# esw0116/DynaVSR

Measured on AMD Instinct MI355X. Metric: inner-loop frames/sec/GPU (EDVR-M x4, 5x3x180x320): forward leg = BASELINE.json configs[1]; the inner MAML step and the per-frame pipeline are `inner_step` / `per_frame_pipeline`, higher is better.
Workload: dtype f32; 1 GPU; EDVR-M x4 forward (PCD deformable alignment + TSA fusion + reconstruction), clips of 1x5x3x180x320 -> 3x720x1280 (BASELINE.json configs[1]); one step = 2 clip(s) per GPU, one per HIP stream (adapt.super_resolve_video); clips_in_flight_per_gpu=2

## Files before the change

dynavsr_amd/csrc/conv2d_wino5.hip:

```cpp
#include <type_traits>

#include "common.h"
#include "kernels.h"
#include "small_grid.h"

namespace dvsr {

#ifdef DVSR_CONV_TRACE
#define W5_STAMP(i)                                                                                       \
  do {                                                                                                    \
    if (a.trace && threadIdx.x == 0) a.trace[(size_t)blockIdx.x * 64 + (i)] = __builtin_readcyclecounter(); \
  } while (0)
#else
#define W5_STAMP(i) \
  do {              \
  } while (0)
#endif

typedef float w5f2 __attribute__((ext_vector_type(2)));
typedef __bf16 w5bf8 __attribute__((ext_vector_type(8)));
typedef __bf16 w5bf2 __attribute__((ext_vector_type(2)));
typedef unsigned w5u4 __attribute__((ext_vector_type(4)));

constexpr int W5_PCH = 18 * 2 * 3 * 256;

template <int TC>
struct Wino5Shape {
  static constexpr int CC = 8, NTILE = 32, TRW = NTILE / TC, NT = 768;
  static constexpr int OH = 4 * TRW, OW = 4 * TC;
  static constexpr int IH = OH + 2, RP = OW + 8, GR = RP / 4;
  static constexpr int NG = CC * IH * GR;
  static constexpr int NI = (NG + NT - 1) / NT;
  static constexpr int RAWPAD = NI * NT * 4;
  static constexpr int VIMG = 36 * 3 * 32 * 4;
  static constexpr int XCH = 6 * 16 * 64 * 4;
  static constexpr int LOOP = 2 * RAWPAD + 2 * VIMG;
  static constexpr size_t LDS_BYTES = (size_t)(LOOP > XCH ? LOOP : XCH) * sizeof(float);
};

constexpr int w5_waitcnt(int vm, int lgkm) { return (vm & 15) | (7 << 4) | ((lgkm & 15) << 8) | ((vm >> 4) << 14); }

__device__ __forceinline__ unsigned w5_cvt_pk(float a, float b) {
  return __builtin_bit_cast(unsigned, __builtin_convertvector(w5f2{a, b}, w5bf2));
}
__device__ __forceinline__ void w5_dma16(__amdgpu_buffer_rsrc_t rs, float* lds, unsigned voff, unsigned soff) {
  __builtin_amdgcn_raw_ptr_buffer_load_lds(rs, (__attribute__((address_space(3))) void*)lds, 16, voff, soff, 0, 0);
}
__device__ __forceinline__ __amdgpu_buffer_rsrc_t w5_rsrc(const float* base, int num_records) {
  return __builtin_amdgcn_make_buffer_rsrc(const_cast<float*>(base), 0, num_records, 0x00020000);
}

__global__ void pack_weights_wino5_kernel(PackTable t) {
  const PackEntry& e = t.e[blockIdx.y];
  if (e.layout != PackLayout::WINO_F4) return;
  __bf16* const P16 = reinterpret_cast<__bf16*>(e.P);
  const size_t total = (size_t)e.ncb * e.nchunks * 512;
  constexpr double G[6][3] = {{1.0 / 4, 0, 0},          {-1.0 / 6, -1.0 / 6, -1.0 / 6}, {-1.0 / 6, 1.0 / 6, -1.0 / 6},
                              {1.0 / 24, 1.0 / 12, 1.0 / 6}, {1.0 / 24, -1.0 / 12, 1.0 / 6}, {0, 0, 1}};
  for (size_t i = blockIdx.x * (size_t)blockDim.x + threadIdx.x; i < total; i += (size_t)gridDim.x * blockDim.x) {
    const int c8 = (int)(i & 7), col = (int)((i >> 3) & 63);
    const size_t ck = i >> 9;
    const int k = (int)(ck % e.nchunks), cb = (int)(ck / e.nchunks);
    const int co = cb * 64 + col, ci = k * 8 + c8;
    double g[3][3];
    const bool ok = co < e.Cout && ci < e.Ctot;
    const float* src = !e.wt ? e.w + ((size_t)co * (e.w_ctot ? e.w_ctot : e.Ctot) + (e.w_ctot ? e.w_coff : 0) + ci) * 9
                             : e.w + ((size_t)ci * e.w_ctot + e.w_coff + co) * 9;
#pragma unroll
    for (int tap = 0; tap < 9; ++tap) g[tap / 3][tap % 3] = ok ? (double)src[e.wt ? 8 - tap : tap] : 0.0;
    double c[6][3];
#pragma unroll
    for (int xi = 0; xi < 6; ++xi)
#pragma unroll
      for (int b = 0; b < 3; ++b) c[xi][b] = G[xi][0] * g[0][b] + G[xi][1] * g[1][b] + G[xi][2] * g[2][b];
    const int mh = col >> 5, c32 = col & 31;
    __bf16* dst = P16 + ck * (size_t)(2 * W5_PCH) + (size_t)mh * 1536 + (size_t)c32 * 8 + c8;
#pragma unroll
    for (int xi = 0; xi < 6; ++xi)
#pragma unroll
      for (int nu = 0; nu < 6; ++nu) {
        const float u = (float)(c[xi][0] * G[nu][0] + c[xi][1] * G[nu][1] + c[xi][2] * G[nu][2]);
        const __bf16 h = (__bf16)u;
        const float r1 = u - (float)h;
        const __bf16 m = (__bf16)r1;
        const __bf16 l = (__bf16)(r1 - (float)m);
        __bf16* d = dst + (size_t)(xi * 3 + (nu >> 1)) * 3072;
        if (nu & 1) { d[512] = m; d[768] = h; d[1024] = l; }
        else { d[0] = h; d[256] = m; d[1280] = l; }
      }
  }
}

int pack_weights_wino5_run(const PackTable& t, hipStream_t st) {
  hipLaunchKernelGGL(pack_weights_wino5_kernel, dim3(64, t.n), dim3(256), 0, st, t);
  return check_launch("pack_weights_wino5_kernel");
}

template <int TC, bool RES, bool R16, bool PRE>
__global__ __launch_bounds__(1024) void conv2d_wino5_kernel(ConvK2 a) {
  static_assert(!PRE || (R16 && !RES), "the addend is read by the sixteen-reader epilogue, never beside a residual");
  using Sh = Wino5Shape<TC>;
  constexpr int IH = Sh::IH, RP = Sh::RP, GR = Sh::GR;
  constexpr int CHF = IH * RP;
  constexpr int QF = 768 * 4;
  extern __shared__ __attribute__((aligned(16))) float smem[];
  float* const raw0 = smem;
  unsigned* const vimg0 = reinterpret_cast<unsigned*>(smem + 2 * Sh::RAWPAD);

  const int id = blockIdx.x;
  const int q_ = id >> 3;
  const int cbi = q_ % a.ncb;
  const int j_ = q_ / a.ncb;
  const int tile = (id & 7) * a.tiles_per_xcd + j_;
  if (j_ >= a.tiles_per_xcd || tile >= a.ntiles) return;
  const int tx_ = tile % a.tiles_x;
  const int t2 = tile / a.tiles_x;
  const int ty_ = t2 % a.tiles_y;
  const int n = t2 / a.tiles_y;
  const int oy0 = ty_ * Sh::OH, ox0 = tx_ * Sh::OW;

  const int tid = threadIdx.x, lane = tid & 63;
  const int wave = __builtin_amdgcn_readfirstlane(tid >> 6);
  const int lo = lane & 31, hi = lane >> 5;
  const size_t HW = (size_t)a.H * a.W;
  auto fence = [&]() __attribute__((always_inline)) { __builtin_amdgcn_sched_barrier(0); };
  auto lds_barrier = [&]() __attribute__((always_inline)) {
    asm volatile("s_waitcnt lgkmcnt(0)" ::: "memory");
    __builtin_amdgcn_s_barrier();
    asm volatile("" ::: "memory");
  };
  W5_STAMP(0);
#ifdef DVSR_CONV_TRACE
  if (a.trace && threadIdx.x == 0) a.trace[(size_t)blockIdx.x * 64 + 60] = __builtin_amdgcn_s_memrealtime();
#endif

  auto read16 = [&](int m) __attribute__((always_inline)) {
    int le = lane;
    asm volatile("" : "+v"(le));
    const int rq_r = wave & 3, cp_r = wave >> 2;
    const float* const xr = smem + (rq_r * 64 + le) * 4 + cp_r;
    const int lo_e = le & 31, hi_e = le >> 5;
    const int trow_e = lo_e / TC, tcol_e = lo_e - trow_e * TC;
    const int oy = oy0 + 4 * trow_e, ox = ox0 + 4 * tcol_e;
    const size_t HWo = (size_t)a.Ho * a.Wo;
    const float slope = a.act == ACT_LRELU ? 0.1f : (a.act == ACT_RELU ? 0.f : 1.f);
    const float* bias = wset_ptr(a.bias, a.b_gs, n, a.wdiv);
    const int co0 = cbi * 64 + m * 32 + 8 * rq_r + 4 * hi_e + cp_r;
    f32x4 pr[4];
    if constexpr (PRE) {
      const bool live = oy < a.Ho && ox < a.Wo && co0 < a.Cout;
      const float* pre = a.pre + (size_t)(n / a.pre_bdiv) * a.pre_bs + (size_t)co0 * HWo + (size_t)oy * a.Wo + ox;
#pragma unroll
      for (int i = 0; i < 4; ++i)
        pr[i] = (live && oy + i < a.Ho) ? *reinterpret_cast<const f32x4*>(pre + (size_t)i * a.Wo) : f32x4{0.f, 0.f, 0.f, 0.f};
    }
    float y[4][4];
#pragma unroll
    for (int j = 0; j < 4; ++j) {
      float z[6];
#pragma unroll
      for (int x = 0; x < 6; ++x) z[x] = xr[(x * 16 + j * 4) * 256];
      const float sa = z[1] + z[2], da = z[1] - z[2];
      const float sb = z[3] + z[4], db = z[3] - z[4];
      y[0][j] = z[0] + sa + sb;
      y[1][j] = __builtin_fmaf(2.f, db, da);
      y[2][j] = __builtin_fmaf(4.f, sb, sa);
      y[3][j] = __builtin_fmaf(8.f, db, da) + z[5];
    }
    const bool px_ok = oy < a.Ho && ox < a.Wo;
    const int nrow = a.Ho - oy < 4 ? a.Ho - oy : 4;
    if (px_ok && co0 < a.Cout) {
      const float b0 = bias ? bias[co0] : 0.f;
      const size_t base = ((size_t)n * a.Cout + co0) * HWo + (size_t)oy * a.Wo + ox;
      f32x4 rr[4];
      if constexpr (RES) {
#pragma unroll
        for (int i = 0; i < 4; ++i)
          rr[i] = i < nrow ? *reinterpret_cast<const f32x4*>(a.res + base + (size_t)i * a.Wo) : f32x4{0.f, 0.f, 0.f, 0.f};
      }
#pragma unroll
      for (int i = 0; i < 4; ++i) {
        if (i >= nrow) break;
        f32x4 v;
#pragma unroll
        for (int j = 0; j < 4; ++j) {
          float v0 = y[i][j] + b0;
          if constexpr (PRE) v0 += pr[i][j];
          v[j] = fmaxf(v0, v0 * slope);
        }
        if constexpr (RES) v += rr[i];
        *reinterpret_cast<f32x4*>(a.y + base + (size_t)i * a.Wo) = v;
      }
    }
  };

  if (wave >= 12) {
    const int pw = wave - 12, ptid = tid - 768;
    const float* x0n = a.x0 + (size_t)n * a.x0_bs;
    const float* x1n = a.c1 ? a.x1 + (size_t)(n / a.x1_bdiv) * a.x1_bs : x0n;
    static_assert(IH * GR * 4 == 720, "a channel quad is 720 groups");
    unsigned hoff[3];
#pragma unroll
    for (int jj = 0; jj < 3; ++jj) {
      const int L = jj * 256 + ptid;
      const int cq = L / (IH * GR), rr = L - cq * (IH * GR);
      const int iy = rr / GR, g = rr - iy * GR;
      const int gy = oy0 - 1 + iy, gx = ox0 - 4 + 4 * g;
      const bool live = L < 4 * IH * GR;
      const bool ok = live && (unsigned)gy < (unsigned)a.H && (unsigned)gx < (unsigned)a.W;
      hoff[jj] = ok ? (unsigned)(((size_t)cq * HW + (size_t)gy * a.W + gx) * 4) : 0x80000000u;
      if (live && !ok) {
#pragma unroll
        for (int bb = 0; bb < 4; ++bb) *reinterpret_cast<f32x4*>(raw0 + (bb >> 1) * Sh::RAWPAD + (bb & 1) * QF + L * 4) = f32x4{0.f, 0.f, 0.f, 0.f};
      }
    }
    const unsigned chunk_bytes = (unsigned)(Sh::CC * HW * 4), quad_bytes = (unsigned)(4 * HW * 4);
    auto issue_raw = [&](int k) __attribute__((always_inline)) {
      const bool live = k < a.nchunks;
      const bool second = k * Sh::CC >= a.c0;
      const unsigned soff = live ? (unsigned)(second ? k - a.c0 / Sh::CC : k) * chunk_bytes : 0u;
      const __amdgpu_buffer_rsrc_t rs = w5_rsrc(second ? x1n : x0n, live ? 0x7fffffff : 0);
      float* dst = raw0 + (k & 1) * Sh::RAWPAD + 256 * pw;
#pragma unroll
      for (int jj = 0; jj < 3; ++jj) {
        w5_dma16(rs, dst + jj * 1024, hoff[jj], soff);
        w5_dma16(rs, dst + QF + jj * 1024, hoff[jj], soff + quad_bytes);
      }
    };
    const int ptile = 8 * pw + (lane & 7), ppair = (lane >> 3) & 3;
    const int trow_t = ptile / TC, tcol_t = ptile - trow_t * TC;
    const int pch = 2 * ppair + hi;
    const float* prd = raw0 + (pch >> 2) * QF + (pch & 3) * CHF + 4 * trow_t * RP + 4 * tcol_t;
    unsigned* vw12 = vimg0 + (hi ? 2 : 1) * 6 * 384 + ptile * 4 + ppair;
    unsigned* vw34 = vimg0 + (hi ? 4 : 3) * 6 * 384 + ptile * 4 + ppair;
    unsigned* vw05 = vimg0 + (hi ? 5 : 0) * 6 * 384 + ptile * 4 + ppair;
    auto ld_row = [&](float (&d)[6], int row) __attribute__((always_inline)) {
      const float* p = prd + row * RP;
      const w5f2 l2 = *reinterpret_cast<const w5f2*>(p + 2);
      const f32x4 m4 = *reinterpret_cast<const f32x4*>(p + 4);
      const w5f2 h2 = *reinterpret_cast<const w5f2*>(p + 8);
      d[0] = l2[1]; d[1] = m4[0]; d[2] = m4[1]; d[3] = m4[2]; d[4] = m4[3]; d[5] = h2[0];
    };
    auto colpass = [&](const float (&r)[6], float (&v)[6]) __attribute__((always_inline)) {
      v[0] = __builtin_fmaf(4.f, r[0], __builtin_fmaf(-5.f, r[2], r[4]));
      v[5] = __builtin_fmaf(4.f, r[1], __builtin_fmaf(-5.f, r[3], r[5]));
      const float e1 = __builtin_fmaf(-4.f, r[2], r[4]), o1 = __builtin_fmaf(-4.f, r[1], r[3]);
      v[1] = e1 + o1; v[2] = e1 - o1;
      const float e2 = r[4] - r[2], o2 = r[3] - r[1];
      v[3] = __builtin_fmaf(2.f, o2, e2); v[4] = __builtin_fmaf(-2.f, o2, e2);
    };
    auto finish_pair = [&](const float (&ra)[6], const float (&rb)[6], unsigned* vw) __attribute__((always_inline)) {
      float va[6], vb[6];
      colpass(ra, va);
      colpass(rb, vb);
#pragma unroll
      for (int v = 0; v < 6; ++v) {
        const auto s0 = __builtin_amdgcn_permlane32_swap(__builtin_bit_cast(unsigned, va[v]), __builtin_bit_cast(unsigned, vb[v]), false, false);
        const unsigned u0 = s0[0], u1 = s0[1];
        const float v0 = __builtin_bit_cast(float, u0), v1 = __builtin_bit_cast(float, u1);
        const unsigned h = w5_cvt_pk(v0, v1);
        const float r0 = v0 - __builtin_bit_cast(float, h << 16), r1 = v1 - __builtin_bit_cast(float, h & 0xffff0000u);
        const unsigned m = w5_cvt_pk(r0, r1);
        const float q0 = r0 - __builtin_bit_cast(float, m << 16), q1 = r1 - __builtin_bit_cast(float, m & 0xffff0000u);
        unsigned* d = vw + v * 384;
#ifdef W5_NOVW
        d[0] = h ^ m ^ w5_cvt_pk(q0, q1);
#else
        d[0] = h; d[128] = m; d[256] = w5_cvt_pk(q0, q1);
#endif
      }
    };
    auto produce = [&]() __attribute__((always_inline)) {
      float d0[6], d1[6], d2[6], d3[6], d4[6], d5[6];
      ld_row(d1, 1); ld_row(d2, 2); ld_row(d3, 3); ld_row(d4, 4);
      ld_row(d0, 0); ld_row(d5, 5);
      float ra[6], rb[6];
#pragma unroll
      for (int j = 0; j < 6; ++j) {
        const float e = __builtin_fmaf(-4.f, d2[j], d4[j]), o = __builtin_fmaf(-4.f, d1[j], d3[j]);
        ra[j] = e + o; rb[j] = e - o;
      }
      finish_pair(ra, rb, vw12);
      fence();
#pragma unroll
      for (int j = 0; j < 6; ++j) {
        const float e = d4[j] - d2[j], o = d3[j] - d1[j];
        ra[j] = __builtin_fmaf(2.f, o, e); rb[j] = __builtin_fmaf(-2.f, o, e);
      }
      finish_pair(ra, rb, vw34);
      fence();
#pragma unroll
      for (int j = 0; j < 6; ++j) {
        ra[j] = __builtin_fmaf(4.f, d0[j], __builtin_fmaf(-5.f, d2[j], d4[j]));
        rb[j] = __builtin_fmaf(4.f, d1[j], __builtin_fmaf(-5.f, d3[j], d5[j]));
      }
      finish_pair(ra, rb, vw05);
    };
    issue_raw(0);
    issue_raw(1);
    __builtin_amdgcn_s_waitcnt(w5_waitcnt(6, 0));
    __builtin_amdgcn_s_barrier();
    asm volatile("" ::: "memory");
    produce();
    __builtin_amdgcn_s_waitcnt(w5_waitcnt(0, 0));
    __builtin_amdgcn_s_barrier();
    asm volatile("" ::: "memory");
    int vstep = Sh::VIMG, rstep = Sh::RAWPAD;
    vw12 += vstep; vw34 += vstep; vw05 += vstep; prd += rstep;
    __builtin_amdgcn_s_setprio(3);
    for (int k = 0; k < a.nchunks; ++k) {

#ifndef W5_NODMA
      issue_raw(k + 2);
#endif
#ifndef W5_NOPROD
      if (k + 1 < a.nchunks) produce();
#endif
      __builtin_amdgcn_s_waitcnt(w5_waitcnt(0, 0));
      __builtin_amdgcn_s_barrier();
      asm volatile("" ::: "memory");
      vw12 -= vstep; vw34 -= vstep; vw05 -= vstep; prd -= rstep;
      vstep = -vstep; rstep = -rstep;
    }
    if constexpr (R16) {
      __builtin_amdgcn_s_setprio(0);
      lds_barrier();
      lds_barrier(); read16(0);
      lds_barrier();
      lds_barrier(); read16(1);
    } else {
      lds_barrier(); lds_barrier(); lds_barrier(); lds_barrier();
    }
    return;
  }
  {
    const int cxi = wave % 6, cmh = wave / 6;
    f32x16 acc[6];
#pragma unroll
    for (int v = 0; v < 6; ++v)
#pragma unroll
      for (int r = 0; r < 16; ++r) acc[v][r] = 0.f;
    const float* wp_cb = wset_ptr(a.wp, a.w_gs, n, a.wdiv) + (size_t)cbi * a.nchunks * W5_PCH;
    const __amdgpu_buffer_rsrc_t wrsrc = w5_rsrc(wp_cb, -1);
    const unsigned avoff = (unsigned)(lane * 16);
    const int asb = (cxi * 3 * 2 + cmh) * 3072;
    f32x4 AF[3];
    auto gldA = [&](auto g_, int k) __attribute__((always_inline)) {
      constexpr int G = decltype(g_)::value;
#ifdef W5_NOA
      if (k > 0 || G > 2) return;
#endif
      const int soff = k * (W5_PCH * 4) + asb + (G / 3) * 6144 + (G % 3) * 1024;
      AF[G % 3] = __builtin_bit_cast(f32x4, __builtin_amdgcn_raw_buffer_load_b128(wrsrc, (int)avoff, soff, 0));
    };
    auto blend = [&](f32x4& x, const f32x4& l, bool keep) __attribute__((always_inline)) {
#pragma unroll
      for (int r = 0; r < 4; ++r) x[r] = keep ? x[r] : l[r];
    };
    const unsigned* vrd = vimg0 + cxi * 6 * 384 + lo * 4;
    const unsigned* vrd_lh = vrd + (hi ? 0 : 256);
    const unsigned* vrd_hl = vrd + (hi ? 256 : 0);
    w5u4 BF[2];
    auto ldB = [&](auto f_) __attribute__((always_inline)) {
      constexpr int F = decltype(f_)::value, NU = F / 3, W = F % 3;
      if constexpr (W == 0) BF[F & 1] = *reinterpret_cast<const w5u4*>(vrd + NU * 384);
      else if constexpr (W == 1) BF[F & 1] = *reinterpret_cast<const w5u4*>(vrd + NU * 384 + 128);
      else if constexpr (NU & 1) BF[F & 1] = *reinterpret_cast<const w5u4*>(vrd_hl + NU * 384);
      else BF[F & 1] = *reinterpret_cast<const w5u4*>(vrd_lh + NU * 384);
    };
    auto mma = [&](f32x16& c, const f32x4& av, const w5u4& bv) __attribute__((always_inline)) {
#ifdef W5_NOMMA
      c[0] += av[0] * __builtin_bit_cast(float, bv[0]);
      return;
#endif
      c = __builtin_amdgcn_mfma_f32_32x32x16_bf16(__builtin_bit_cast(w5bf8, av), __builtin_bit_cast(w5bf8, bv), c, 0, 0, 0);
    };
    static_for<0, 3>([&](auto g_) __attribute__((always_inline)) { gldA(g_, 0); });
    __builtin_amdgcn_s_barrier();
    asm volatile("" ::: "memory");
    __builtin_amdgcn_s_barrier();
    asm volatile("" ::: "memory");
    int vstep = Sh::VIMG;
    for (int k = 0; k < a.nchunks; ++k) {
      ldB(std::integral_constant<int, 0>{}); ldB(std::integral_constant<int, 1>{});
      const int knext = k + 1 < a.nchunks ? k + 1 : k;
      static_for<0, 18>([&](auto f_) __attribute__((always_inline)) {
        constexpr int F = decltype(f_)::value, NU = F / 3, I = F % 3;
        constexpr int XS = NU & 1;
        mma(acc[NU], AF[XS], BF[F & 1]);
#ifdef W5_NOBR
        if constexpr (false)
#else
        if constexpr (F + 2 < 18)
#endif
          ldB(std::integral_constant<int, (F + 2 < 18 ? F + 2 : 0)>{});
        if constexpr (I == 1) {
          blend(AF[XS], AF[2], (NU & 1) ? hi != 0 : hi == 0);
          if constexpr ((NU & 1) && NU < 5) gldA(std::integral_constant<int, 3 * ((NU < 5 ? NU : 1) / 2) + 5>{}, k);
          if constexpr (NU == 5) gldA(std::integral_constant<int, 2>{}, knext);
        }
        if constexpr (I == 2) {
          if constexpr (NU < 4) gldA(std::integral_constant<int, 3 * ((NU < 4 ? NU : 0) / 2) + 3 + (NU & 1)>{}, k);
          else gldA(std::integral_constant<int, (NU & 1)>{}, knext);
        }
        fence();
      });
      lds_barrier();
      if (k < 16) W5_STAMP(3 + k);
      vrd += vstep; vrd_lh += vstep; vrd_hl += vstep;
      vstep = -vstep;
    }
  W5_STAMP(40);

  int lane_e = lane;
  asm volatile("" : "+v"(lane_e));
  f32x16 Z[4];
#pragma unroll
  for (int r = 0; r < 16; ++r) {
    const float sa = acc[1][r] + acc[2][r], da = acc[1][r] - acc[2][r];
    const float sb = acc[3][r] + acc[4][r], db = acc[3][r] - acc[4][r];
    Z[0][r] = acc[0][r] + sa + sb;
    Z[1][r] = __builtin_fmaf(2.f, db, da);
    Z[2][r] = __builtin_fmaf(4.f, sb, sa);
    Z[3][r] = __builtin_fmaf(8.f, db, da) + acc[5][r];
  }
  float* const xw = smem + (cxi * 16 * 64 + lane_e) * 4;
  const int rq_r = wave & 3, cp_r = wave >> 2;
  const float* const xr = smem + (rq_r * 64 + lane_e) * 4 + cp_r * 2;
  const int lo_e = lane_e & 31, hi_e = lane_e >> 5;
  const int trow_e = lo_e / TC, tcol_e = lo_e - trow_e * TC;
  const int oy = oy0 + 4 * trow_e, ox = ox0 + 4 * tcol_e;
  const size_t HWo = (size_t)a.Ho * a.Wo;
  const float slope = a.act == ACT_LRELU ? 0.1f : (a.act == ACT_RELU ? 0.f : 1.f);
  const float* bias = wset_ptr(a.bias, a.b_gs, n, a.wdiv);
  W5_STAMP(50);
  lds_barrier();
  W5_STAMP(51);
#pragma unroll 1
  for (int m = 0; m < 2; ++m) {
    if (cmh == m) {
#pragma unroll
      for (int j = 0; j < 4; ++j)
#pragma unroll
        for (int rq = 0; rq < 4; ++rq)
          *reinterpret_cast<f32x4*>(xw + (j * 4 + rq) * 256) = f32x4{Z[j][4 * rq], Z[j][4 * rq + 1], Z[j][4 * rq + 2], Z[j][4 * rq + 3]};
    }
    W5_STAMP(52 + 4 * m);
    lds_barrier();
    W5_STAMP(53 + 4 * m);
    if constexpr (R16) read16(m);
    else if (wave < 8) {
      const int co0 = cbi * 64 + m * 32 + 8 * rq_r + 4 * hi_e + 2 * cp_r;
      float y[2][4][4];
#pragma unroll
      for (int j = 0; j < 4; ++j) {
        w5f2 z[6];
#pragma unroll
        for (int x = 0; x < 6; ++x) z[x] = *reinterpret_cast<const w5f2*>(xr + (x * 16 + j * 4) * 256);
#pragma unroll
        for (int c = 0; c < 2; ++c) {
          const float sa = z[1][c] + z[2][c], da = z[1][c] - z[2][c];
          const float sb = z[3][c] + z[4][c], db = z[3][c] - z[4][c];
          y[c][0][j] = z[0][c] + sa + sb;
          y[c][1][j] = __builtin_fmaf(2.f, db, da);
          y[c][2][j] = __builtin_fmaf(4.f, sb, sa);
          y[c][3][j] = __builtin_fmaf(8.f, db, da) + z[5][c];
        }
      }
      const bool px_ok = oy < a.Ho && ox < a.Wo;
      const int nrow = a.Ho - oy < 4 ? a.Ho - oy : 4;
      if (px_ok && co0 < a.Cout) {
        const bool two = co0 + 1 < a.Cout;
        const float b0 = bias ? bias[co0] : 0.f, b1 = (bias && two) ? bias[co0 + 1] : 0.f;
#pragma unroll
        for (int i = 0; i < 4; ++i)
#pragma unroll
          for (int j = 0; j < 4; ++j) {
            const float v0 = y[0][i][j] + b0, v1 = y[1][i][j] + b1;
            y[0][i][j] = fmaxf(v0, v0 * slope);
            y[1][i][j] = fmaxf(v1, v1 * slope);
          }
        if (a.ps == 0) {
#pragma unroll
          for (int c = 0; c < 2; ++c) {
            if (c == 1 && !two) break;
            const size_t base = ((size_t)n * a.Cout + co0 + c) * HWo + (size_t)oy * a.Wo + ox;
            if constexpr (RES) {
              f32x4 rr[4];
#pragma unroll
              for (int i = 0; i < 4; ++i)
                rr[i] = i < nrow ? *reinterpret_cast<const f32x4*>(a.res + base + (size_t)i * a.Wo) : f32x4{0.f, 0.f, 0.f, 0.f};
#pragma unroll
              for (int i = 0; i < 4; ++i) {
                if (i >= nrow) break;
                const f32x4 v = f32x4{y[c][i][0], y[c][i][1], y[c][i][2], y[c][i][3]} + rr[i];
                *reinterpret_cast<f32x4*>(a.y + base + (size_t)i * a.Wo) = v;
              }
            } else {
#pragma unroll
              for (int i = 0; i < 4; ++i) {
                if (i >= nrow) break;
                *reinterpret_cast<f32x4*>(a.y + base + (size_t)i * a.Wo) = f32x4{y[c][i][0], y[c][i][1], y[c][i][2], y[c][i][3]};
              }
            }
          }
        } else {
          const int cq = co0 >> 2, dy = (co0 >> 1) & 1;
          float* dst = a.y + (((size_t)n * (a.Cout >> 2) + cq) * (2 * a.Ho) + (2 * oy + dy)) * (size_t)(2 * a.Wo) + 2 * ox;
#pragma unroll
          for (int i = 0; i < 4; ++i) {
            if (i >= nrow) break;
            float* d = dst + (size_t)(2 * i) * (2 * a.Wo);
            *reinterpret_cast<f32x4*>(d) = f32x4{y[0][i][0], y[1][i][0], y[0][i][1], y[1][i][1]};
            *reinterpret_cast<f32x4*>(d + 4) = f32x4{y[0][i][2], y[1][i][2], y[0][i][3], y[1][i][3]};
          }
        }
      }
    }
    W5_STAMP(54 + 4 * m);
    if (m == 0) lds_barrier();
    W5_STAMP(55 + 4 * m);
  }
#ifdef DVSR_CONV_TRACE
  W5_STAMP(41);
  __builtin_amdgcn_s_waitcnt(0);
  W5_STAMP(42);
  if (a.trace && threadIdx.x == 0) {
    a.trace[(size_t)blockIdx.x * 64 + 61] = __builtin_amdgcn_s_memrealtime();
    a.trace[(size_t)blockIdx.x * 64 + 63] = __builtin_amdgcn_s_getreg((4) | (0 << 6) | (31 << 11));
    a.trace[(size_t)blockIdx.x * 64 + 62] = __builtin_amdgcn_s_getreg((20) | (0 << 6) | (31 << 11));
  }
#endif
  }
}

template <int TC>
static int launch_wino5(ConvK2 k, hipStream_t st) {
  using Sh = Wino5Shape<TC>;
  auto kern = k.pre ? conv2d_wino5_kernel<TC, false, true, true>
                    : (k.res ? conv2d_wino5_kernel<TC, true, true, false> : conv2d_wino5_kernel<TC, false, false, false>);
  static PerDeviceOnce attr_once, attr_once_r, attr_once_p;
  set_dyn_lds_once(attr_once, (const void*)conv2d_wino5_kernel<TC, false, false, false>, Sh::LDS_BYTES);
  set_dyn_lds_once(attr_once_r, (const void*)conv2d_wino5_kernel<TC, true, true, false>, Sh::LDS_BYTES);
  set_dyn_lds_once(attr_once_p, (const void*)conv2d_wino5_kernel<TC, false, true, true>, Sh::LDS_BYTES);
  k.tiles_x = ceil_div(k.Wo, Sh::OW); k.tiles_y = ceil_div(k.Ho, Sh::OH); k.ntiles = k.tiles_x * k.tiles_y * k.N;
  k.ncb = ceil_div(k.Cout, 64);
  k.tiles_per_xcd = ceil_div(k.ntiles, 8);
  k.nitems = k.tiles_per_xcd * 8 * k.ncb;
  hipLaunchKernelGGL(kern, dim3(k.nitems), dim3(1024), Sh::LDS_BYTES, st, k);
  return check_launch("conv2d_wino5_kernel");
}

int conv2d_wino5_launch(const ConvK2& k, int th, hipStream_t st) {
  return th == 16 ? launch_wino5<8>(k, st) : launch_wino5<16>(k, st);
}

}
```

Measured before the change: 266.0 frames/s.

## Restructure Winograd output exchange so both M-halves write per round with vector LDS reads

Reorganizes the LDS exchange image for the Winograd F(4,3) output transform. Both M-halves now write four-record units each round, where before each half waited for its own round. Readers fetch f32x4 records holding all four transform rows in one load instead of strided scalar or float2 loads. The second round's write is moved after the barrier so it overlaps the first round's epilogue, and non-pixel-shuffle convs now use the 16-wave reader variant. An asm register pin is added inside the accumulator transform to steer register allocation. This adds layout bookkeeping in a new header with compile-time coverage checks, and risks LDS bank conflicts and higher register pressure.

```diff
diff --git a/dynavsr_amd/csrc/conv2d_wino5.hip b/dynavsr_amd/csrc/conv2d_wino5.hip
--- a/dynavsr_amd/csrc/conv2d_wino5.hip
+++ b/dynavsr_amd/csrc/conv2d_wino5.hip
@@ -3,6 +3,7 @@
 #include "common.h"
 #include "kernels.h"
 #include "small_grid.h"
+#include "wino5_exchange.h"
 
 namespace dvsr {
 
@@ -134,18 +135,18 @@
   if (a.trace && threadIdx.x == 0) a.trace[(size_t)blockIdx.x * 64 + 60] = __builtin_amdgcn_s_memrealtime();
 #endif
 
-  auto read16 = [&](int m) __attribute__((always_inline)) {
+  auto read16 = [&](int t) __attribute__((always_inline)) {
     int le = lane;
     asm volatile("" : "+v"(le));
-    const int rq_r = wave & 3, cp_r = wave >> 2;
-    const float* const xr = smem + (rq_r * 64 + le) * 4 + cp_r;
+    const int m_r = w5x::r16_mh(wave), rq_r = w5x::r16_rq(wave, t), c_r = w5x::r16_c(wave);
+    const float* const xr = smem + w5x::rec(m_r, rq_r, 0, c_r, le);
     const int lo_e = le & 31, hi_e = le >> 5;
     const int trow_e = lo_e / TC, tcol_e = lo_e - trow_e * TC;
     const int oy = oy0 + 4 * trow_e, ox = ox0 + 4 * tcol_e;
     const size_t HWo = (size_t)a.Ho * a.Wo;
     const float slope = a.act == ACT_LRELU ? 0.1f : (a.act == ACT_RELU ? 0.f : 1.f);
     const float* bias = wset_ptr(a.bias, a.b_gs, n, a.wdiv);
-    const int co0 = cbi * 64 + m * 32 + 8 * rq_r + 4 * hi_e + cp_r;
+    const int co0 = cbi * 64 + w5x::cout_of(m_r, rq_r, hi_e, c_r);
     f32x4 pr[4];
     if constexpr (PRE) {
       const bool live = oy < a.Ho && ox < a.Wo && co0 < a.Cout;
@@ -154,18 +155,18 @@
       for (int i = 0; i < 4; ++i)
         pr[i] = (live && oy + i < a.Ho) ? *reinterpret_cast<const f32x4*>(pre + (size_t)i * a.Wo) : f32x4{0.f, 0.f, 0.f, 0.f};
     }
+    f32x4 z[6];
+#pragma unroll
+    for (int x = 0; x < 6; ++x) z[x] = *reinterpret_cast<const f32x4*>(xr + x * (w5x::NC * w5x::NLANE * w5x::REC_F));
     float y[4][4];
 #pragma unroll
     for (int j = 0; j < 4; ++j) {
-      float z[6];
-#pragma unroll
-      for (int x = 0; x < 6; ++x) z[x] = xr[(x * 16 + j * 4) * 256];
-      const float sa = z[1] + z[2], da = z[1] - z[2];
-      const float sb = z[3] + z[4], db = z[3] - z[4];
-      y[0][j] = z[0] + sa + sb;
+      const float sa = z[1][j] + z[2][j], da = z[1][j] - z[2][j];
+      const float sb = z[3][j] + z[4][j], db = z[3][j] - z[4][j];
+      y[0][j] = z[0][j] + sa + sb;
       y[1][j] = __builtin_fmaf(2.f, db, da);
       y[2][j] = __builtin_fmaf(4.f, sb, sa);
-      y[3][j] = __builtin_fmaf(8.f, db, da) + z[5];
+      y[3][j] = __builtin_fmaf(8.f, db, da) + z[5][j];
     }
     const bool px_ok = oy < a.Ho && ox < a.Wo;
     const int nrow = a.Ho - oy < 4 ? a.Ho - oy : 4;
@@ -412,8 +413,6 @@
     }
   W5_STAMP(40);
 
-  int lane_e = lane;
-  asm volatile("" : "+v"(lane_e));
   f32x16 Z[4];
 #pragma unroll
   for (int r = 0; r < 16; ++r) {
@@ -423,10 +422,18 @@
     Z[1][r] = __builtin_fmaf(2.f, db, da);
     Z[2][r] = __builtin_fmaf(4.f, sb, sa);
     Z[3][r] = __builtin_fmaf(8.f, db, da) + acc[5][r];
+    if ((r & 3) == 3 && r < 15) {
+      auto rec = [&](int q) __attribute__((always_inline)) { return f32x4{Z[0][q], Z[1][q], Z[2][q], Z[3][q]}; };
+      asm volatile("" : "+v"(acc[1][r + 1]), "+v"(acc[1][r + 2]), "+v"(acc[1][r + 3]), "+v"(acc[1][r + 4]),
+                        "+v"(acc[3][r + 1]), "+v"(acc[3][r + 2]), "+v"(acc[3][r + 3]), "+v"(acc[3][r + 4])
+                   : "v"(rec(r - 3)), "v"(rec(r - 2)), "v"(rec(r - 1)), "v"(rec(r)));
+    }
   }
-  float* const xw = smem + (cxi * 16 * 64 + lane_e) * 4;
-  const int rq_r = wave & 3, cp_r = wave >> 2;
-  const float* const xr = smem + (rq_r * 64 + lane_e) * 4 + cp_r * 2;
+  int lane_e = lane;
+  asm volatile("" : "+v"(lane_e));
+  static_assert(Sh::XCH == w5x::IMG_F, "the exchange image is one round's four units");
+  float* const xw = smem + w5x::rec(cmh, 0, cxi, 0, lane_e);
+  const int m_r = w5x::r8_mh(wave), c_r = w5x::r8_c(wave);
   const int lo_e = lane_e & 31, hi_e = lane_e >> 5;
   const int trow_e = lo_e / TC, tcol_e = lo_e - trow_e * TC;
   const int oy = oy0 + 4 * trow_e, ox = ox0 + 4 * tcol_e;
@@ -436,35 +443,41 @@
   W5_STAMP(50);
   lds_barrier();
   W5_STAMP(51);
+  auto xwrite = [&](auto t_) __attribute__((always_inline)) {
+    constexpr int T = decltype(t_)::value;
+#pragma unroll
+    for (int rqb = 0; rqb < 2; ++rqb)
+#pragma unroll
+      for (int c = 0; c < 4; ++c) {
+        const int r = 4 * (2 * T + rqb) + c;
+        *reinterpret_cast<f32x4*>(xw + rqb * w5x::UNIT_F + c * (w5x::NLANE * w5x::REC_F)) = f32x4{Z[0][r], Z[1][r], Z[2][r], Z[3][r]};
+      }
+  };
+  xwrite(std::integral_constant<int, 0>{});
 #pragma unroll 1
   for (int m = 0; m < 2; ++m) {
-    if (cmh == m) {
-#pragma unroll
-      for (int j = 0; j < 4; ++j)
-#pragma unroll
-        for (int rq = 0; rq < 4; ++rq)
-          *reinterpret_cast<f32x4*>(xw + (j * 4 + rq) * 256) = f32x4{Z[j][4 * rq], Z[j][4 * rq + 1], Z[j][4 * rq + 2], Z[j][4 * rq + 3]};
-    }
     W5_STAMP(52 + 4 * m);
     lds_barrier();
     W5_STAMP(53 + 4 * m);
     if constexpr (R16) read16(m);
     else if (wave < 8) {
-      const int co0 = cbi * 64 + m * 32 + 8 * rq_r + 4 * hi_e + 2 * cp_r;
+      const int rq_r = w5x::r8_rq(wave, m);
+      const float* const xr = smem + w5x::rec(m_r, rq_r, 0, c_r, lane_e);
+      const int co0 = cbi * 64 + w5x::cout_of(m_r, rq_r, hi_e, c_r);
       float y[2][4][4];
 #pragma unroll
-      for (int j = 0; j < 4; ++j) {
-        w5f2 z[6];
-#pragma unroll
-        for (int x = 0; x < 6; ++x) z[x] = *reinterpret_cast<const w5f2*>(xr + (x * 16 + j * 4) * 256);
-#pragma unroll
-        for (int c = 0; c < 2; ++c) {
-          const float sa = z[1][c] + z[2][c], da = z[1][c] - z[2][c];
-          const float sb = z[3][c] + z[4][c], db = z[3][c] - z[4][c];
-          y[c][0][j] = z[0][c] + sa + sb;
+      for (int c = 0; c < 2; ++c) {
+        f32x4 z[6];
+#pragma unroll
+        for (int x = 0; x < 6; ++x) z[x] = *reinterpret_cast<const f32x4*>(xr + (x * w5x::NC + c) * (w5x::NLANE * w5x::REC_F));
+#pragma unroll
+        for (int j = 0; j < 4; ++j) {
+          const float sa = z[1][j] + z[2][j], da = z[1][j] - z[2][j];
+          const float sb = z[3][j] + z[4][j], db = z[3][j] - z[4][j];
+          y[c][0][j] = z[0][j] + sa + sb;
           y[c][1][j] = __builtin_fmaf(2.f, db, da);
           y[c][2][j] = __builtin_fmaf(4.f, sb, sa);
-          y[c][3][j] = __builtin_fmaf(8.f, db, da) + z[5][c];
+          y[c][3][j] = __builtin_fmaf(8.f, db, da) + z[5][j];
         }
       }
       const bool px_ok = oy < a.Ho && ox < a.Wo;
@@ -520,6 +533,7 @@
     W5_STAMP(54 + 4 * m);
     if (m == 0) lds_barrier();
     W5_STAMP(55 + 4 * m);
+    if (m == 0) xwrite(std::integral_constant<int, 1>{});
   }
 #ifdef DVSR_CONV_TRACE
   W5_STAMP(41);
@@ -538,9 +552,11 @@
 static int launch_wino5(ConvK2 k, hipStream_t st) {
   using Sh = Wino5Shape<TC>;
   auto kern = k.pre ? conv2d_wino5_kernel<TC, false, true, true>
-                    : (k.res ? conv2d_wino5_kernel<TC, true, true, false> : conv2d_wino5_kernel<TC, false, false, false>);
-  static PerDeviceOnce attr_once, attr_once_r, attr_once_p;
+                    : (k.res ? conv2d_wino5_kernel<TC, true, true, false>
+                             : (k.ps ? conv2d_wino5_kernel<TC, false, false, false> : conv2d_wino5_kernel<TC, false, true, false>));
+  static PerDeviceOnce attr_once, attr_once_r, attr_once_p, attr_once_16;
   set_dyn_lds_once(attr_once, (const void*)conv2d_wino5_kernel<TC, false, false, false>, Sh::LDS_BYTES);
+  set_dyn_lds_once(attr_once_16, (const void*)conv2d_wino5_kernel<TC, false, true, false>, Sh::LDS_BYTES);
   set_dyn_lds_once(attr_once_r, (const void*)conv2d_wino5_kernel<TC, true, true, false>, Sh::LDS_BYTES);
   set_dyn_lds_once(attr_once_p, (const void*)conv2d_wino5_kernel<TC, false, true, true>, Sh::LDS_BYTES);
   k.tiles_x = ceil_div(k.Wo, Sh::OW); k.tiles_y = ceil_div(k.Ho, Sh::OH); k.ntiles = k.tiles_x * k.tiles_y * k.N;
diff --git a/dynavsr_amd/csrc/wino5_exchange.h b/dynavsr_amd/csrc/wino5_exchange.h
--- /dev/null
+++ b/dynavsr_amd/csrc/wino5_exchange.h
@@ -0,0 +1,66 @@
+#pragma once
+
+namespace dvsr {
+namespace w5x {
+
+constexpr int NXI = 6, NC = 4, NLANE = 64, REC_F = 4;
+constexpr int UNIT_F = NXI * NC * NLANE * REC_F;
+constexpr int ROUND_UNITS = 4, ROUNDS = 2;
+constexpr int IMG_F = ROUND_UNITS * UNIT_F;
+
+__host__ __device__ constexpr int round_of(int rq) { return rq >> 1; }
+__host__ __device__ constexpr int unit_pos(int mh, int rq) { return 2 * mh + (rq & 1); }
+__host__ __device__ constexpr int rec(int mh, int rq, int xi, int c, int lane) {
+  return unit_pos(mh, rq) * UNIT_F + ((xi * NC + c) * NLANE + lane) * REC_F;
+}
+__host__ __device__ constexpr int cout_of(int mh, int rq, int hi, int c) { return 32 * mh + 8 * rq + 4 * hi + c; }
+
+__host__ __device__ constexpr int r16_mh(int wave) { return wave >> 3; }
+__host__ __device__ constexpr int r16_rq(int wave, int t) { return 2 * t + ((wave >> 2) & 1); }
+__host__ __device__ constexpr int r16_c(int wave) { return wave & 3; }
+__host__ __device__ constexpr int r8_mh(int wave) { return wave >> 2; }
+__host__ __device__ constexpr int r8_rq(int wave, int t) { return 2 * t + ((wave >> 1) & 1); }
+__host__ __device__ constexpr int r8_c(int wave) { return 2 * (wave & 1); }
+
+namespace check {
+constexpr bool round_is_a_partition(int t) {
+  bool seen[IMG_F / REC_F] = {};
+  for (int mh = 0; mh < 2; ++mh)
+    for (int rq = 2 * t; rq < 2 * t + 2; ++rq)
+      for (int xi = 0; xi < NXI; ++xi)
+        for (int c = 0; c < NC; ++c)
+          for (int lane = 0; lane < NLANE; ++lane) {
+            const int f = rec(mh, rq, xi, c, lane);
+            if (round_of(rq) != t || f < 0 || f % REC_F || f + REC_F > IMG_F || seen[f / REC_F]) return false;
+            seen[f / REC_F] = true;
+          }
+  for (bool s : seen)
+    if (!s) return false;
+  return true;
+}
+constexpr bool readers_cover(bool pairs) {
+  int hits[64] = {};
+  for (int t = 0; t < ROUNDS; ++t) {
+    bool unit_c[2][4][NC] = {};
+    for (int wave = 0; wave < (pairs ? 8 : 16); ++wave)
+      for (int k = 0; k < (pairs ? 2 : 1); ++k) {
+        const int mh = pairs ? r8_mh(wave) : r16_mh(wave), rq = pairs ? r8_rq(wave, t) : r16_rq(wave, t);
+        const int c = (pairs ? r8_c(wave) : r16_c(wave)) + k;
+        if (mh > 1 || rq > 3 || c >= NC || round_of(rq) != t || unit_c[mh][rq][c]) return false;
+        unit_c[mh][rq][c] = true;
+        for (int hi = 0; hi < 2; ++hi) ++hits[cout_of(mh, rq, hi, c)];
+      }
+  }
+  for (int h : hits)
+    if (h != 1) return false;
+  return true;
+}
+static_assert(round_is_a_partition(0) && round_is_a_partition(1), "a round's four units tile the exchange image exactly");
+static_assert(readers_cover(false), "sixteen readers: every cout of the block exactly once");
+static_assert(readers_cover(true), "eight pair readers: every cout of the block exactly once");
+static_assert(r8_c(0) % 2 == 0 && r8_c(1) % 2 == 0, "a pair is (even cout, odd cout): PixelShuffle(2)'s dx");
+static_assert(cout_of(1, 3, 1, 3) == 63 && cout_of(0, 0, 0, 0) == 0, "MFMA row layout");
+}
+
+}
+}
```

Result: faster. 269.8 frames/s, median of 6 (+1.5%).
